# erwincoumans/tiny-differentiable-simulator

Measured on AMD Instinct MI355X. Metric: env-steps/sec, higher is better.
Workload: dtype f64

## Files before the change

tiny-differentiable-simulator_amd/csrc/tds_oct.hip:

```cpp
#include <hip/hip_runtime.h>
#include <stdlib.h>

#include "tds_device_model.h"
#include "tds_kernels.h"
#include "tds_lanes.h"
#include "tds_oct_windows.h"
#include "tds_step_shared.h"

#ifdef TDS_OCT_PROF
#ifndef TDS_OCT_PROF_WG
#define TDS_OCT_PROF_WG 3
#endif
__device__ unsigned long long tds_oct_prof_buf[64];
__device__ unsigned long long tds_oct_prof_clk[64];
__device__ unsigned long long tds_oct_prof_wg[3 * 2048];
__device__ int tds_oct_prof_iter = 500;
#define OCT_STAMP(k, pin)                                                                       \
  do {                                                                                          \
    unsigned long long t_;                                                                      \
    auto p_ = (pin);        \
    asm volatile("s_memtime %0\n\ts_waitcnt lgkmcnt(0)" : "=s"(t_), "+v"(p_)::"memory");        \
    if (prof_on) prof_t[k] = t_;                                                                \
  } while (0)
#define OCT_BAR_T(k)       \
  do {                     \
    OCT_STAMP(k, tid);     \
    OCT_BAR();             \
    OCT_STAMP((k) + 1, tid); \
  } while (0)
#define OCT_BAR_W(k, first)                                                                     \
  do {                                                                                          \
    unsigned long long a_, b_;                                                                  \
    asm volatile("s_memtime %0\n\ts_waitcnt lgkmcnt(0)" : "=s"(a_), "+v"(tid)::"memory");       \
    OCT_BAR();                                                                                  \
    asm volatile("s_memtime %0\n\ts_waitcnt lgkmcnt(0)" : "=s"(b_), "+v"(tid)::"memory");       \
    if (prof_on && (first)) {                                                                   \
      prof_t[k] = a_;                                                                           \
      prof_t[(k) + 1] = b_;                                                                     \
    } else if (prof_on) {                                                                       \
      prof_t[(k) + 2] += b_ - a_;                                                               \
    }                                                                                           \
  } while (0)
#else
#define OCT_STAMP(k, pin) do { } while (0)
#define OCT_BAR_T(k) OCT_BAR()
#define OCT_BAR_W(k, first) OCT_BAR()
#endif

#ifdef TDS_OCT_MARKS
#define OCT_MARK(name) asm volatile("; OCTMARK " name ::: "memory")
#else
#define OCT_MARK(name) do { } while (0)
#endif

#ifndef TDS_OCT_SD_LATE
#define TDS_OCT_SD_LATE 1
#endif
#ifndef TDS_OCT_CARRY
#define TDS_OCT_CARRY 1
#endif
#ifndef TDS_OCT_TOP_EARLY
#define TDS_OCT_TOP_EARLY 1
#endif
#ifndef TDS_OCT_SPLIT_LOOP
#define TDS_OCT_SPLIT_LOOP 0
#endif

namespace {

#define OCT_SYNC()                                             \
  do {                                                         \
    __builtin_amdgcn_fence(__ATOMIC_ACQ_REL, "wavefront");     \
    __builtin_amdgcn_wave_barrier();                           \
  } while (0)

template <int CTRL>
__device__ __forceinline__ double oct_dpp(double v) {
  const int l = __double2loint(v), h = __double2hiint(v);
  const int lo = __builtin_amdgcn_update_dpp(0, l, CTRL, 0xF, 0xF, true);
  const int hi = __builtin_amdgcn_update_dpp(0, h, CTRL, 0xF, 0xF, true);
  return __hiloint2double(hi, lo);
}
template <int CTRL>
__device__ __forceinline__ float oct_dpp(float v) {
  return __int_as_float(__builtin_amdgcn_update_dpp(0, __float_as_int(v), CTRL, 0xF, 0xF, true));
}
template <typename T>
__device__ __forceinline__ T pair_other(T v) { return oct_dpp<0xB1>(v); }
template <int K, typename T>
__device__ __forceinline__ T pair_bcast(T v) { return oct_dpp<(K == 0 ? 0xA0 : 0xF5)>(v); }
template <typename T>
__device__ __forceinline__ T oct_sum(T v) {
  asm volatile("" : "+v"(v));
  v += oct_dpp<0xB1>(v);
  v += oct_dpp<0x4E>(v);
  v += oct_dpp<0x141>(v);
  return v;
}
template <int K>
__device__ __forceinline__ double oct_bcast(double v) {
  const double t = __builtin_amdgcn_update_dpp(0.0, v, 0x150 + K, 0xF, 0x3, false);
  return __builtin_amdgcn_update_dpp(t, v, 0x150 + 8 + K, 0xF, 0xC, false);
}
template <int K>
__device__ __forceinline__ float oct_bcast(float v) {
  const int b = __float_as_int(v);
  const int t = __builtin_amdgcn_update_dpp(0, b, 0x150 + K, 0xF, 0x3, false);
  return __int_as_float(__builtin_amdgcn_update_dpp(t, b, 0x150 + 8 + K, 0xF, 0xC, false));
}

struct OctOff {
  int lcw, legf, swl, qdp, fac, win, xs, cp, stride;
};
struct OctLds {
  static constexpr int LCW = 6;
  static constexpr int ZW = 14;
  static constexpr int Z_B = 10, Z_A = 11, Z_G = 12, Z_HL = 13;
  static constexpr int NCP = 17;
};
__host__ __device__ inline OctOff oct_layout(int in_dim) {
  OctOff o;
  int at = in_dim + 4;
  at = (at + 1) & ~1;
  o.lcw = at;  at += 8 * OctLds::LCW;
  o.legf = at; at += 4 * 3;
  o.swl = at;  at += 8 * 6;
  o.qdp = at;  at += 8;
  o.fac = at;  at += 28;
  o.win = at;  at += 2 * 8 * OctLds::ZW;
  o.xs = at;   at += 3 * OctLds::NCP + 1;
  o.cp = at;   at += 5 * OctLds::NCP + 1;
  at = (at + 1) & ~1;
  while ((((at * 2) & 63) % 8) != 0 || ((at * 2) & 63) == 0 || ((at * 2) & 63) == 32) at += 2;
  o.stride = at;
  return o;
}

struct OctKernArgs {
  const void *mdl, *x_in;
  void *y_out;
  const void *actions;
  void *x_feedback, *obs_out;
  TdsStepCtl ctl;
  int n_envs;
  OctOff O;
};
using TB = TdsOctTab;
constexpr int TDS_OCT_PRIO = 1;

#define OCT_ST(v, p) (*(p) = (v))
#define OCT_BAR()                                                                        \
  do {                                                                                   \
    if constexpr (W2) asm volatile("s_waitcnt lgkmcnt(0)\n\ts_barrier" ::: "memory");    \
    else OCT_SYNC();                                                                     \
  } while (0)

template <typename T, typename TR, bool LOOP, int BUILD>
__device__ __forceinline__ void oct_body(const DevModel<T> *__restrict__ mdl_arg, const TR *x_in, TR *__restrict__ y_out,
                                         const TR *__restrict__ actions, TR *x_feedback ,
                                         TR *__restrict__ obs_out, const TdsStepCtl &ctl_arg, int n_envs, const OctOff &O) {
  extern __shared__ __align__(16) unsigned char tds_oct_smem[];
  T *const sm = reinterpret_cast<T *>(tds_oct_smem);
#ifdef TDS_OCT_PROF
  if (threadIdx.x == 0 && blockIdx.x < 2048) {
    unsigned long long c_;
    asm volatile("s_memrealtime %0\n\ts_waitcnt lgkmcnt(0)" : "=s"(c_)::"memory");
    tds_oct_prof_wg[3 * blockIdx.x] = c_;
  }
#endif
  constexpr bool W2 = BUILD >= 2;
  constexpr bool BATCH_SCHUR = LOOP && BUILD == 3;
  constexpr bool SD_LATE = LOOP && (BUILD == 2 || BUILD == 3) && TDS_OCT_SD_LATE != 0;
  constexpr bool CARRY = LOOP && BUILD == 3 && TDS_OCT_CARRY != 0;
  constexpr bool TOP_EARLY = LOOP && BUILD == 3 && TDS_OCT_TOP_EARLY != 0;
  constexpr bool SPLIT_LOOP = CARRY || TOP_EARLY || (LOOP && BUILD == 3 && TDS_OCT_SPLIT_LOOP != 0);
  constexpr int nq = 14, nd = 14, adim = 8, in_dim = nq + nd + adim + 3, w_obs = nq + nd + 2;
  constexpr int NT = W2 ? 128 : 64;
  T *const CT = sm + 8 * O.stride;
  {
    const int t = threadIdx.x;
    constexpr int TN = (TB::TOTAL + NT - 1) / NT, XN = (in_dim + 7) / 8;
    T tv[TN], xv[XN];
#pragma unroll
    for (int k = 0; k < TN; ++k) {
      const int i = t + k * NT;
      tv[k] = i < TB::TOTAL ? mdl_arg->oct_tab[i] : T(0);
    }
    const int lane0 = t & 7, grp0 = (t & 63) >> 3, env0 = blockIdx.x * 8 + grp0;
    const bool valid0 = env0 < n_envs && t < 64;
#pragma unroll
    for (int k = 0; k < XN; ++k) {
      const int i = lane0 + 8 * k;
      const bool act = actions != nullptr && i >= nq + nd && i < nq + nd + adim;
      xv[k] = (!valid0 || i >= in_dim) ? T(0) : act ? (T)actions[(size_t)env0 * adim + (i - nq - nd)] : (T)x_in[(size_t)env0 * in_dim + i];
    }
#pragma unroll
    for (int k = 0; k < TN; ++k) {
      const int i = t + k * NT;
      if (i < TB::TOTAL) CT[i] = tv[k];
    }
    if (t < 64) {
      T *const xr = sm + grp0 * O.stride;
#pragma unroll
      for (int k = 0; k < XN; ++k) {
        const int i = lane0 + 8 * k;
        if (i < in_dim) xr[i] = xv[k];
      }
      if (lane0 < 4) xr[in_dim + lane0] = T(0);
    }
    if constexpr (W2) __syncthreads();
    else OCT_SYNC();
  }
  const int nsteps = LOOP ? ctl_arg.nsub : 1;
  T next_act = T(0);
  int act_blk = 0, y_slot = 0, o_slot = 0;
  if constexpr (LOOP) {
    if (ctl_arg.act_pool != nullptr && ctl_arg.act_blocks > 0) act_blk = (ctl_arg.act_first + 1) % ctl_arg.act_blocks;
    if (ctl_arg.y_ring != nullptr && ctl_arg.y_slots > 0) y_slot = ctl_arg.y_first % ctl_arg.y_slots;
    if (ctl_arg.obs_ring != nullptr && ctl_arg.obs_slots > 0) o_slot = ctl_arg.obs_first % ctl_arg.obs_slots;
  }
  const int act_slot = (int)(CT + (threadIdx.x & 7) * TB::LSTR)[TB::ACT];
  struct Carried { T q, qd, rq[6], rqd[6]; };
  struct TopConsts { T S[6], rotf, nax[3], nn[6], xt[3], ipose, stiff, damp, act_lim, xt_ident, base_t[3], grav[3], kp, kd, max_force; };
  auto carry_load = [&](const T *xr_, int lane_, Carried &c) {
    c.q = xr_[6 + lane_];
    c.qd = xr_[nq + 6 + lane_];
#pragma unroll
    for (int r = 0; r < 6; ++r) {
      c.rq[r] = xr_[r];
      c.rqd[r] = xr_[nq + r];
    }
  };
  auto top_request = [&](const T *xr_, const T *CL_, TopConsts &t) {
#pragma unroll
    for (int k = 0; k < 6; ++k) t.S[k] = CL_[TB::S + k];
    t.rotf = CL_[TB::ROTF];
#pragma unroll
    for (int k = 0; k < 3; ++k) t.nax[k] = CL_[TB::NAX + k];
#pragma unroll
    for (int k = 0; k < 6; ++k) t.nn[k] = CL_[TB::NN + k];
#pragma unroll
    for (int k = 0; k < 3; ++k) t.xt[k] = CL_[TB::XT + 9 + k];
    t.ipose = CL_[TB::IPOSE];
    t.stiff = CL_[TB::STIFF];
    t.damp = CL_[TB::DAMP];
    t.act_lim = CT[TB::SC + TB::ACTION_LIMIT];
    t.xt_ident = CT[TB::SC + TB::XT_IDENT];
#pragma unroll
    for (int k = 0; k < 3; ++k) {
      t.base_t[k] = CT[TB::SC + TB::BASE_T + k];
      t.grav[k] = CT[TB::SC + TB::GRAV + k];
    }
    t.kp = xr_[nq + nd + adim];
    t.kd = xr_[nq + nd + adim + 1];
    t.max_force = xr_[nq + nd + adim + 2];
  };
  Carried car = {};
  TopConsts tc = {};
  if constexpr (CARRY || TOP_EARLY) {
    const int lane_ = threadIdx.x & 7;
    const T *const xr_ = sm + ((threadIdx.x & 63) >> 3) * O.stride;
    if constexpr (CARRY) carry_load(xr_, lane_, car);
    if constexpr (TOP_EARLY) top_request(xr_, CT + lane_ * TB::LSTR, tc);
  }
  auto step_body = [&](auto rolec, const int it) {
  constexpr int ROLE = decltype(rolec)::value;
  const __attribute__((address_space(4))) char *ka_seg = (const __attribute__((address_space(4))) char *)__builtin_amdgcn_kernarg_segment_ptr();
  int tid = threadIdx.x;
  if constexpr (LOOP) asm volatile("" : "+s"(ka_seg), "+v"(tid));
  const int wv = ROLE < 2 ? ROLE : (W2 ? __builtin_amdgcn_readfirstlane(tid >> 6) : 0);
  const bool is_main = !W2 || wv == 0, is_help = !W2 || wv == 1;
  if constexpr (W2 && TDS_OCT_PRIO != 0) {
    if (BUILD != 4 && wv == 0) __builtin_amdgcn_s_setprio(3);
    else __builtin_amdgcn_s_setprio(0);
  }
  (void)is_main;
  (void)is_help;
#ifdef TDS_OCT_PROF
  unsigned long long prof_t[56] = {};
  const bool prof_on = blockIdx.x == TDS_OCT_PROF_WG && it == tds_oct_prof_iter;
  if (it == 0 && tid == 0 && blockIdx.x < 2048) {
    unsigned long long c_;
    asm volatile("s_memrealtime %0\n\ts_waitcnt lgkmcnt(0)" : "=s"(c_)::"memory");
    tds_oct_prof_wg[3 * blockIdx.x + 1] = c_;
  }
  if (blockIdx.x == TDS_OCT_PROF_WG && it < 32 && tid == 0) {
    unsigned long long c0_, c1_;
    asm volatile("s_memtime %0\n\ts_memrealtime %1\n\ts_waitcnt lgkmcnt(0)" : "=s"(c0_), "=s"(c1_)::"memory");
    tds_oct_prof_clk[2 * it] = c0_;
    tds_oct_prof_clk[2 * it + 1] = c1_;
  }
#endif
  const int lane = tid & 7;
  const int grp = (tid & 63) >> 3;
  const int env = blockIdx.x * 8 + grp;
  const bool valid = env < n_envs;
  T *const E = sm + grp * O.stride;
  T *const xr = E;
  const int leg = lane >> 1, pos = lane & 1;
  const int dq = 6 + lane;
  const T *const CL = CT + lane * TB::LSTR;
  typename TdsCtlRef<LOOP>::type ctl = TdsCtlRef<LOOP>::get(ctl_arg, ka_seg + __builtin_offsetof(OctKernArgs, ctl));
  const T dt = CT[TB::SC + TB::DT];
  const int pgs_iters = (int)CT[TB::SC + TB::PGS_ITERATIONS];
  const bool last = it == nsteps - 1;
  OCT_STAMP(0, tid);

  T q, qd, tau;
  T Sl[6], R[9], p[3], sw[6], v[6], a0[6];
  T R5[9], P[3], A4[3], A5[3], pA3[3], pA4[3], pA5[3], v5[6], a5[6];
  T Lc[6], l10, id0, id1, sq0, sq1, my_id, my_sq, Ls[15], ids[6], sq_ids[6], qd_new, qdr_new[6];
  T Cb, Cr[6], It[10];
  T u = T(0), urm = T(0);
  T u_init = T(0), urm_init = T(0);
  T sw_mu = T(0), sw_rest = T(0), sw_cap = T(0), sw_hip = T(0);
  int na = 0, NA = 0;

  auto root_frame = [&](const T *rq, const T *bt, T sx, T cx, T sy, T cy, T sz, T cz) {
    R5[0] = cy * cz;                 R5[1] = -cy * sz;                R5[2] = sy;
    R5[3] = sx * sy * cz + cx * sz;  R5[4] = cx * cz - sx * sy * sz;  R5[5] = -sx * cy;
    R5[6] = sx * sz - cx * sy * cz;  R5[7] = cx * sy * sz + sx * cz;  R5[8] = cx * cy;
    P[0] = rq[0] + bt[0];
    P[1] = rq[1] + bt[1];
    P[2] = rq[2] + bt[2];
    A4[0] = T(0); A4[1] = cx; A4[2] = sx;
    A5[0] = sy; A5[1] = -sx * cy; A5[2] = cx * cy;
    pA3[0] = T(0); pA3[1] = P[2]; pA3[2] = -P[1];
    cross3(P, A4, pA4);
// ... 154 lines not shown
      }
      T Rl[9], pl[3], r[3];
      mat3_mul(Rq, Rp, Rl);
      mat3_mulv(Rq, tp, r);
#pragma unroll
      for (int k = 0; k < 3; ++k) pl[k] = pq[k] + r[k];
      mat3_mul(R5, Rl, R);
      mat3_mulv(R5, pl, r);
      p[0] = P[0] + r[0];
      p[1] = P[1] + r[1];
      p[2] = P[2] + r[2];
      mat3_mulv(R, Sl, sw);
      mat3_mulv(R, Sl + 3, sw + 3);
      T c[3];
      cross3(p, sw, c);
      sw[3] += c[0];
      sw[4] += c[1];
      sw[5] += c[2];
      T vJ[6];
#pragma unroll
      for (int k = 0; k < 6; ++k) vJ[k] = sw[k] * qd;
#pragma unroll
      for (int k = 0; k < 6; ++k) {
        const T sh = pair_bcast<0>(vJ[k]);
        v[k] = v5[k] + (vJ[k] + (take ? sh : T(0)));
      }
      T cb[6];
      cross3(v, vJ, cb);
      T c1[3], c2[3];
      cross3(v, vJ + 3, c1);
      cross3(v + 3, vJ, c2);
      cb[3] = c1[0] + c2[0];
      cb[4] = c1[1] + c2[1];
      cb[5] = c1[2] + c2[2];
#pragma unroll
      for (int k = 0; k < 6; ++k) {
        const T sh = pair_bcast<0>(cb[k]);
        a0[k] = a5[k] + (cb[k] + (take ? sh : T(0)));
      }
    }
    OCT_MARK("main_publish_kin");
    {
      T *const swl = E + O.swl + lane * 6;
#pragma unroll
      for (int k = 0; k < 6; ++k) swl[k] = sw[k];
      if constexpr (W2) {
        T *const kin = E + O.win + 8 * OctLds::ZW + lane * 12;
#pragma unroll
        for (int k = 0; k < 9; ++k) kin[k] = R[k];
#pragma unroll
        for (int k = 0; k < 3; ++k) kin[9 + k] = p[k];
      }
    }
    OCT_MARK("main_kin_end");
    OCT_STAMP(1, sw[5]);
  };

  const int ystr = ctl.y_stride;
  const int out_dim = (int)CT[TB::SC + TB::OUTPUT_DIM];
  const int nv = (int)CT[TB::SC + TB::NUM_VISUALS];
  auto y_where = [&](TR *&yo, TR *&yo2, int &yend, int &yend2) {
    int ys = y_slot;
    asm volatile("" : "+s"(ys));
    yo = nullptr;
    yo2 = nullptr;
    yend = ystr;
    yend2 = out_dim;
    if (LOOP && ctl.y_ring != nullptr) {
      yo = tds_global((TR *)ctl.y_ring) + ((size_t)ys * ctl.ring_envs + env) * ystr;
      if (last && y_out != nullptr) yo2 = y_out + (size_t)env * out_dim;
    } else if (last && y_out != nullptr) {
      yo = y_out + (size_t)env * (LOOP ? out_dim : ystr);
      yend = LOOP ? out_dim : ystr;
    }
  };
  unsigned sig_tok = 0u;

  auto help_np = [&]() {
    OCT_MARK("help_np");
    if constexpr (LOOP) {
      if (it > 0 && ctl.obs_ring != nullptr && ctl.peer_arrive != nullptr)
        sig_tok = tds_peer_count_in(ctl, (o_slot == 0 ? ctl.obs_slots : o_slot) - 1);
      if (ctl.act_pool != nullptr && it + 1 < nsteps && valid)
        next_act = (T)tds_global((const TR *)ctl.act_pool)[((size_t)act_blk * ctl.act_envs + env) * adim + lane];
    }
    if constexpr (W2) {
      const T *const kin = E + O.win + 8 * OctLds::ZW + lane * 12;
#pragma unroll
      for (int k = 0; k < 9; ++k) R[k] = kin[k];
#pragma unroll
      for (int k = 0; k < 3; ++k) p[k] = kin[9 + k];
      const T *const sc = E + O.win + 8 * OctLds::ZW + 96;
      root_frame(xr, CT + TB::SC + TB::BASE_T, sc[0], sc[1], sc[2], sc[3], sc[4], sc[5]);
    }
    {
      T *const cpx = E + O.cp;
      const T n[3] = {CT[TB::SC + TB::PLANE_N], CT[TB::SC + TB::PLANE_N + 1], CT[TB::SC + TB::PLANE_N + 2]};
      const T pc = CT[TB::SC + TB::PLANE_C];
      auto sphere = [&](const T *Rl, const T *pl, const T *loc, T rad, T *pt, T &dist) {
        T ctr[3];
        mat3_mulv(Rl, loc, ctr);
        ctr[0] += pl[0];
        ctr[1] += pl[1];
        ctr[2] += pl[2];
        const T t = -((-dot3(ctr, n)) + pc);
        dist = t - rad;
        pt[0] = ctr[0] - rad * n[0];
        pt[1] = ctr[1] - rad * n[1];
        pt[2] = ctr[2] - rad * n[2];
      };
      T pt0[3], pt1[3], ptt[3], d0, d1, dtt;
      sphere(R, p, CL + TB::CPL0, CL[TB::CPR0], pt0, d0);
      sphere(R, p, CL + TB::CPL1, CL[TB::CPR1], pt1, d1);
      sphere(R5, P, CT + TB::ROOT + TB::R_CPL, CT[TB::ROOT + TB::R_CPR], ptt, dtt);
      const bool act0 = valid && d0 < T(0), act1 = valid && d1 < T(0), actt = valid && dtt < T(0) && CT[TB::ROOT + TB::R_CPR] >= T(0);
      const unsigned long long b0 = __ballot(act0), b1 = __ballot(act1), bt = __ballot(actt);
      const unsigned m0 = (unsigned)((b0 >> (grp * 8)) & 0xFFull), m1 = (unsigned)((b1 >> (grp * 8)) & 0xFFull);
      const unsigned below = (1u << lane) - 1u;
      const int r0 = (actt ? 1 : 0) + __popc(m0 & below) + __popc(m1 & below);
      const int r1 = r0 + (act0 ? 1 : 0);
      if (act0) {
        cpx[0 * OctLds::NCP + r0] = pt0[0];
        cpx[1 * OctLds::NCP + r0] = pt0[1];
        cpx[2 * OctLds::NCP + r0] = pt0[2];
        cpx[3 * OctLds::NCP + r0] = d0;
        cpx[4 * OctLds::NCP + r0] = (T)lane;
      }
      if (act1) {
        cpx[0 * OctLds::NCP + r1] = pt1[0];
        cpx[1 * OctLds::NCP + r1] = pt1[1];
        cpx[2 * OctLds::NCP + r1] = pt1[2];
        cpx[3 * OctLds::NCP + r1] = d1;
        cpx[4 * OctLds::NCP + r1] = (T)lane;
      }
      if (actt && lane == 0) {
        cpx[0 * OctLds::NCP] = ptt[0];
        cpx[1 * OctLds::NCP] = ptt[1];
        cpx[2 * OctLds::NCP] = ptt[2];
        cpx[3 * OctLds::NCP] = dtt;
        cpx[4 * OctLds::NCP] = T(8);
      }
      na = (actt ? 1 : 0) + __popc(m0) + __popc(m1);
#pragma unroll
      for (int g = 0; g < 8; ++g) {
        const int c = __popc((unsigned)((b0 >> (g * 8)) & 0xFFull)) + __popc((unsigned)((b1 >> (g * 8)) & 0xFFull)) + (int)((bt >> (g * 8)) & 1ull);
        NA = c > NA ? c : NA;
      }
      if constexpr (W2) {
        if ((tid & 63) == 0) sm[in_dim + 3] = (T)NA;
      }
    }
    OCT_STAMP(8, na);
  };
  auto help_poses = [&]() {
    OCT_MARK("help_signal_poses");
    if constexpr (LOOP) {
      if (ctl.act_pool != nullptr && !last) xr[nq + nd + lane] = next_act;
      if (it > 0 && ctl.obs_ring != nullptr) {
        if (ctl.peer_arrive != nullptr) tds_peer_finish(ctl, (o_slot == 0 ? ctl.obs_slots : o_slot) - 1, sig_tok);
        else tds_signal_slot(ctl, (o_slot == 0 ? ctl.obs_slots : o_slot) - 1);
      }
    }
    TR *yo, *yo2;
    int yend, yend2;
    y_where(yo, yo2, yend, yend2);
    (void)yend;
    (void)yend2;
    if (valid && yo != nullptr && nv > 0) {
      auto pose_out = [&](const T *Rl, const T *pl, const T *vx, int k) {
        T Ro[9], po[3], qo[4];
        mat3_mul(Rl, vx, Ro);
        mat3_mulv(Rl, vx + 9, po);
        matrix_to_quat(Ro, qo);
        TR *o = yo + (nq + nd) + 7 * k;
        OCT_ST((TR)(pl[0] + po[0]), &o[0]);
        OCT_ST((TR)(pl[1] + po[1]), &o[1]);
        OCT_ST((TR)(pl[2] + po[2]), &o[2]);
        OCT_ST((TR)qo[0], &o[3]);
        OCT_ST((TR)qo[1], &o[4]);
        OCT_ST((TR)qo[2], &o[5]);
        OCT_ST((TR)qo[3], &o[6]);
        if (yo2 != nullptr) {
          TR *o2 = yo2 + (nq + nd) + 7 * k;
          OCT_ST((TR)(pl[0] + po[0]), &o2[0]);
          OCT_ST((TR)(pl[1] + po[1]), &o2[1]);
          OCT_ST((TR)(pl[2] + po[2]), &o2[2]);
          OCT_ST((TR)qo[0], &o2[3]);
          OCT_ST((TR)qo[1], &o2[4]);
          OCT_ST((TR)qo[2], &o2[5]);
          OCT_ST((TR)qo[3], &o2[6]);
        }
      };
      pose_out(R, p, CL + TB::VIS, 1 + lane);
      if (lane == 7) pose_out(R5, P, CT + TB::ROOT + TB::R_VIS, 0);
    }
    OCT_MARK("help_np_end");
    OCT_STAMP(9, na);
  };

  auto main_dyn = [&]() {
    auto rigid = [&](const T *Rl, const T *pl, T m, const T *com, const T *Ib, const T *vl, const T *al, T *Ic, T *fc) {
      T cw[3];
      mat3_mulv(Rl, com, cw);
      cw[0] += pl[0];
      cw[1] += pl[1];
      cw[2] += pl[2];
      T RI[9], Iw[9];
      mat3_mul(Rl, Ib, RI);
#pragma unroll
      for (int r = 0; r < 3; ++r)
#pragma unroll
        for (int c = 0; c < 3; ++c) Iw[3 * r + c] = RI[3 * r] * Rl[3 * c] + RI[3 * r + 1] * Rl[3 * c + 1] + RI[3 * r + 2] * Rl[3 * c + 2];
      const T c2 = dot3(cw, cw);
      Ic[0] = Iw[0] + m * (c2 - cw[0] * cw[0]);
      Ic[1] = T(0.5) * (Iw[1] + Iw[3]) - m * cw[0] * cw[1];
      Ic[2] = T(0.5) * (Iw[2] + Iw[6]) - m * cw[0] * cw[2];
      Ic[3] = Iw[4] + m * (c2 - cw[1] * cw[1]);
      Ic[4] = T(0.5) * (Iw[5] + Iw[7]) - m * cw[1] * cw[2];
      Ic[5] = Iw[8] + m * (c2 - cw[2] * cw[2]);
      Ic[6] = m * cw[0];
      Ic[7] = m * cw[1];
      Ic[8] = m * cw[2];
      Ic[9] = m;
      const T *const h = Ic + 6;
      T Iv[6], Ia[6], t3[3];
      sym3_mulv(Ic, vl, Iv);
      cross3(h, vl + 3, t3);
      Iv[0] += t3[0];
      Iv[1] += t3[1];
      Iv[2] += t3[2];
      cross3(h, vl, t3);
      Iv[3] = m * vl[3] - t3[0];
      Iv[4] = m * vl[4] - t3[1];
      Iv[5] = m * vl[5] - t3[2];
      sym3_mulv(Ic, al, Ia);
      cross3(h, al + 3, t3);
      Ia[0] += t3[0];
      Ia[1] += t3[1];
      Ia[2] += t3[2];
      cross3(h, al, t3);
      Ia[3] = m * al[3] - t3[0];
      Ia[4] = m * al[4] - t3[1];
      Ia[5] = m * al[5] - t3[2];
      T u3[3];
      cross3(vl, Iv, fc);
      cross3(vl + 3, Iv + 3, u3);
      fc[0] += u3[0];
      fc[1] += u3[1];
      fc[2] += u3[2];
      cross3(vl, Iv + 3, fc + 3);
#pragma unroll
      for (int k = 0; k < 6; ++k) fc[k] += Ia[k];
    };
    OCT_MARK("main_rigid");
    T Ic[10], fc[6];
    rigid(R, p, CL[TB::MASS], CL + TB::COM, CL + TB::INER, v, a0, Ic, fc);
    T ft[6];
    rigid(R5, P, CT[TB::ROOT + TB::R_MASS], CT + TB::ROOT + TB::R_COM, CT + TB::ROOT + TB::R_INER, v5, a5, It, ft);
    OCT_STAMP(2, ft[5]);
    OCT_MARK("main_totals");
#pragma unroll
    for (int k = 0; k < 10; ++k) It[k] += oct_sum(Ic[k]);
#pragma unroll
    for (int k = 0; k < 6; ++k) ft[k] += oct_sum(fc[k]);
    {
      const T recv = pos == 0 ? T(1) : T(0);
#pragma unroll
      for (int k = 0; k < 6; ++k) fc[k] += recv * pair_bcast<1>(fc[k]);
#pragma unroll
      for (int k = 0; k < 10; ++k) Ic[k] += recv * pair_bcast<1>(Ic[k]);
    }
    OCT_MARK("main_FC");
    T Fc[6];
    times_inertia(Ic, sw, Fc);
    Cb = dot6(sw, fc);
    const T ax3[6] = {T(1), T(0), T(0), pA3[0], pA3[1], pA3[2]}, ax4[6] = {A4[0], A4[1], A4[2], pA4[0], pA4[1], pA4[2]},
            ax5[6] = {A5[0], A5[1], A5[2], pA5[0], pA5[1], pA5[2]};
    Cr[0] = ft[3];
    Cr[1] = ft[4];
    Cr[2] = ft[5];
    Cr[3] = dot6(ax3, ft);
    Cr[4] = dot6(ax4, ft);
    Cr[5] = dot6(ax5, ft);
    T Bm0, Bm1, Cc[6];
    {
      T s0[6];
#pragma unroll
      for (int k = 0; k < 6; ++k) s0[k] = pair_bcast<0>(sw[k]);
      Bm0 = dot6(Fc, s0);
      Bm1 = dot6(Fc, sw);
      Cc[0] = Fc[3];
      Cc[1] = Fc[4];
      Cc[2] = Fc[5];
      Cc[3] = dot6(Fc, ax3);
      Cc[4] = dot6(Fc, ax4);
      Cc[5] = dot6(Fc, ax5);
    }
    OCT_MARK("main_legldl");
    {
      const T b00 = pair_bcast<0>(Bm0);
      const T b10 = pair_bcast<1>(Bm0), b11 = pair_bcast<1>(Bm1);
      sq0 = rsqrt_full<T>(b00);
      id0 = sq0 * sq0;
      l10 = b10 * id0;
      sq1 = rsqrt_full<T>(b11 - l10 * b10);
      id1 = sq1 * sq1;
    }
    my_id = pos == 0 ? id0 : id1;
    my_sq = pos == 0 ? sq0 : sq1;
    {
      T W[6];
      const T m1 = pos == 1 ? l10 : T(0);
#pragma unroll
      for (int r = 0; r < 6; ++r) {
        W[r] = Cc[r] - m1 * pair_bcast<0>(Cc[r]);
        Lc[r] = W[r] * my_id;
      }
      T *const lcw = E + O.lcw + lane * OctLds::LCW;
      T *const wl = E + O.xs + lane * 6;
#pragma unroll
      for (int r = 0; r < 6; ++r) {
        lcw[r] = Lc[r];
        wl[r] = W[r];
      }
      if (pos == 0) {
        T *const lf = E + O.legf + leg * 3;
        lf[0] = l10;
        lf[1] = sq0;
        lf[2] = sq1;
      }
    }
    OCT_STAMP(3, Lc[5]);
  };
  auto main_dyn2 = [&]() {
    OCT_MARK("main_schur");
    const T ax3[6] = {T(1), T(0), T(0), pA3[0], pA3[1], pA3[2]}, ax4[6] = {A4[0], A4[1], A4[2], pA4[0], pA4[1], pA4[2]},
            ax5[6] = {A5[0], A5[1], A5[2], pA5[0], pA5[1], pA5[2]};
    T Sm[21];
    T F3[6], F4[6];
    auto root_block_a1 = [&]() {
      const T m = It[9];
      times_inertia(It, ax3, F3);
      Sm[0] = m;
      Sm[1] = T(0); Sm[2] = m;
      Sm[3] = T(0); Sm[4] = T(0); Sm[5] = m;
      Sm[6] = F3[3]; Sm[7] = F3[4]; Sm[8] = F3[5]; Sm[9] = dot6(ax3, F3);
    };
    auto root_block_a2 = [&]() {
      times_inertia(It, ax4, F4);
      Sm[10] = F4[3]; Sm[11] = F4[4]; Sm[12] = F4[5]; Sm[13] = dot6(ax4, F3); Sm[14] = dot6(ax4, F4);
    };
    auto root_block_b = [&]() {
      T F5[6];
      times_inertia(It, ax5, F5);
      Sm[15] = F5[3]; Sm[16] = F5[4]; Sm[17] = F5[5]; Sm[18] = dot6(ax5, F3); Sm[19] = dot6(ax5, F4); Sm[20] = dot6(ax5, F5);
    };
    {
      const T *const lcw = E + O.lcw;
      const T *const wl = E + O.xs;
      T *const Ssum = E + O.fac;
      const int code = (int)CL[TB::SCHUR];
      if constexpr (BATCH_SCHUR) {
        T la[3][8], wa[3][8];
        int ee[3];
        auto ask = [&](auto pc) {
          constexpr int pass = decltype(pc)::value;
          const int rc = (code >> (6 * pass)) & 63;
          const int r = rc >> 3, rp = rc & 7;
          ee[pass] = (r * (r + 1)) / 2 + rp;
#pragma unroll
          for (int l = 0; l < 8; ++l) {
            la[pass][l] = lcw[l * OctLds::LCW + r];
            wa[pass][l] = wl[l * 6 + rp];
          }
        };
        auto sum = [&](auto pc) {
          constexpr int pass = decltype(pc)::value;
          T acc = T(0);
#pragma unroll
          for (int l = 0; l < 8; ++l) acc += la[pass][l] * wa[pass][l];
          Ssum[ee[pass]] = acc;
        };
        ask(std::integral_constant<int, 0>{});
        __builtin_amdgcn_sched_barrier(0);
        root_block_a1();
        __builtin_amdgcn_sched_barrier(0);
        sum(std::integral_constant<int, 0>{});
        ask(std::integral_constant<int, 1>{});
        __builtin_amdgcn_sched_barrier(0);
        root_block_a2();
        __builtin_amdgcn_sched_barrier(0);
        sum(std::integral_constant<int, 1>{});
        ask(std::integral_constant<int, 2>{});
        __builtin_amdgcn_sched_barrier(0);
        root_block_b();
        __builtin_amdgcn_sched_barrier(0);
        sum(std::integral_constant<int, 2>{});
      } else {
#pragma unroll
        for (int pass = 0; pass < 3; ++pass) {
          const int rc = (code >> (6 * pass)) & 63;
          const int r = rc >> 3, rp = rc & 7;
          const int e = (r * (r + 1)) / 2 + rp;
          T acc = T(0);
#pragma unroll
          for (int l = 0; l < 8; ++l) acc += lcw[l * OctLds::LCW + r] * wl[l * 6 + rp];
          Ssum[e] = acc;
        }
      }
    }
    OCT_MARK("main_Rblock");
    if constexpr (!BATCH_SCHUR) {
      root_block_a1();
      root_block_a2();
      root_block_b();
    }
    OCT_SYNC();
    OCT_MARK("main_ldl6");
    {
      const T *const Ssum = E + O.fac;
      if constexpr (BATCH_SCHUR) {
        T ss[21];
#pragma unroll
        for (int e = 0; e < 21; ++e) ss[e] = Ssum[e];
        __builtin_amdgcn_sched_barrier(0);
#pragma unroll
        for (int e = 0; e < 21; ++e) Sm[e] -= ss[e];
      } else {
#pragma unroll
        for (int e = 0; e < 21; ++e) Sm[e] -= Ssum[e];
      }
      static_for<0, 6>([&](auto kc) {
        constexpr int k = decltype(kc)::value;
        const T rs = rsqrt_full<T>(Sm[(k * (k + 1)) / 2 + k]);
        const T inv = rs * rs;
        sq_ids[k] = rs;
        ids[k] = inv;
        T col[6];
        static_for<k + 1, 6>([&](auto rc) {
          constexpr int r = decltype(rc)::value;
          col[r] = Sm[(r * (r + 1)) / 2 + k];
          Ls[(r * (r - 1)) / 2 + k] = col[r] * inv;
        });
        static_for<k + 1, 6>([&](auto rc) {
          constexpr int r = decltype(rc)::value;
          static_for<k + 1, r + 1>([&](auto cc) {
            constexpr int c = decltype(cc)::value;
            Sm[(r * (r + 1)) / 2 + c] -= Ls[(r * (r - 1)) / 2 + k] * col[c];
          });
        });
      });
    }
    OCT_STAMP(4, Ls[14]);
    OCT_MARK("main_fd");
    if constexpr (W2) {
      T *const fac = E + O.fac;
      OCT_SYNC();
      if (lane == 0) {
#pragma unroll
        for (int k = 0; k < 15; ++k) fac[k] = Ls[k];
#pragma unroll
        for (int k = 0; k < 6; ++k) fac[15 + k] = sq_ids[k];
      }
    }
    OCT_MARK("main_dyn_end");
  };
  auto main_fd = [&]() {
    OCT_MARK("main_fd");
    T y = tau - Cb;
    y -= (pos == 1 ? l10 : T(0)) * pair_bcast<0>(y);
    T yr[6];
#pragma unroll
    for (int r = 0; r < 6; ++r) yr[r] = -Cr[r] - oct_sum(Lc[r] * y);
    static_for<1, 6>([&](auto rc) {
      constexpr int r = decltype(rc)::value;
      static_for<0, r>([&](auto cc) {
        constexpr int c = decltype(cc)::value;
        yr[r] -= Ls[(r * (r - 1)) / 2 + c] * yr[c];
      });
    });
    u = -dt * (y * my_sq);
    T sel = yr[0] * sq_ids[0];
#pragma unroll
    for (int r = 1; r < 6; ++r) sel = lane == r ? yr[r] * sq_ids[r] : sel;
    urm = lane < 6 ? -dt * sel : T(0);
    u_init = u;
    urm_init = urm;
    OCT_STAMP(5, u);
  };
  auto main_sweep_consts = [&]() {
    OCT_SYNC();
    sw_mu = CT[TB::SC + TB::FRICTION];
    sw_rest = CT[TB::SC + TB::RESTITUTION];
    sw_hip = (T)(lane & ~1);
    int cap = 100000;
    asm volatile("" : "+v"(cap));
    sw_cap = (T)cap;
  };
  auto main_get_count = [&]() { NA = __builtin_amdgcn_readfirstlane((int)sm[in_dim + 3]); };
  auto help_get_factors = [&]() {
    const T *const fac = E + O.fac;
#pragma unroll
    for (int k = 0; k < 15; ++k) Ls[k] = fac[k];
#pragma unroll
    for (int k = 0; k < 6; ++k) sq_ids[k] = fac[15 + k];
  };

  struct RowRegs {
    T z0, z1, zr[6];
    int hl;
// ... 352 lines not shown
    OCT_MARK("main_pool_end");
    OCT_STAMP(7, tid);
  };
  auto help_rec = [&]() {
    OCT_MARK("help_rec");
    TR *yo, *yo2;
    int yend, yend2;
    y_where(yo, yo2, yend, yend2);
    if (valid && yo != nullptr && xr[in_dim + 3] == T(0)) {
      y_state(yo, yend);
      if (yo2 != nullptr) y_state(yo2, yend2);
    }
    if constexpr (LOOP) {
      if (ctl.obs_ring != nullptr) {
        const int slot = o_slot;
        const int rf = ctl.ring_flags;
        const bool f32w = (rf & TDS_RING_OBS_F32) != 0 || sizeof(TR) == 4;
        const int np = ctl.peer_arrive != nullptr ? ctl.n_peers : 0;
        const bool rd_only = (rf & TDS_RING_PEER_REWARD_DONE) != 0;
        if (ctl.peer_arrive != nullptr && (rf & TDS_RING_WIDE) != 0 && __all(valid)) {
          const int wl = tid & 63;
          const size_t row0 = ((size_t)slot * ctl.obs_envs + (size_t)blockIdx.x * 8) * (size_t)w_obs;
          const int per_unit = f32w ? 2 : 1;
          const int n_units = (8 * w_obs) / per_unit;
          const unsigned long long *const __attribute__((address_space(4))) *tab =
              (const unsigned long long *const __attribute__((address_space(4))) *)(const __attribute__((address_space(4))) void *)ctl.peer_ring;
          for (int u0 = 0; u0 < n_units; u0 += 64) {
            const int uu = u0 + wl;
            const bool on = uu < n_units;
            unsigned lo = 0u, hi = 0u;
            bool tail = false;
#pragma unroll
            for (int c = 0; c < 2; ++c) {
              if (c < per_unit) {
                const int f = on ? uu * per_unit + c : 0;
                const int e = f / w_obs;
                const int i = f - e * w_obs;
                const int src = i < nq + nd ? i : (i == nq + nd ? in_dim + 2 : in_dim + 1);
                const T vv = i < 2 ? T(0) : sm[e * O.stride + src];
                tail = tail || i >= nq + nd;
                if (f32w) {
                  const unsigned b = (unsigned)__float_as_int((float)vv);
                  if (c == 0) lo = b; else hi = b;
                } else {
                  const double dv = (double)vv;
                  lo = (unsigned)__double2loint(dv);
                  hi = (unsigned)__double2hiint(dv);
                }
              }
            }
            const unsigned long long bits = ((unsigned long long)hi << 32) | (unsigned long long)lo;
            const size_t unit_at = row0 / per_unit + (size_t)uu;
            if (on) __hip_atomic_store(tds_global((unsigned long long *)ctl.obs_ring) + unit_at, bits, __ATOMIC_RELAXED, __HIP_MEMORY_SCOPE_AGENT);
            const bool to_peers = on && (!rd_only || tail);
            for (int p0 = 0; p0 < np; p0 += 4) {
              const unsigned long long *const b0 = tds_global(tab[p0]), *const b1 = tds_global(tab[p0 + 1]), *const b2 = tds_global(tab[p0 + 2]),
                                       *const b3 = tds_global(tab[p0 + 3]);
              const size_t po = (size_t)ctl.peer_off / 8 + unit_at;
              if (to_peers) {
                using G64 = __attribute__((address_space(1))) unsigned long long;
                __hip_atomic_store((G64 *)((unsigned long long *)b0 + po), bits, __ATOMIC_RELAXED, __HIP_MEMORY_SCOPE_SYSTEM);
                if (p0 + 1 < np) __hip_atomic_store((G64 *)((unsigned long long *)b1 + po), bits, __ATOMIC_RELAXED, __HIP_MEMORY_SCOPE_SYSTEM);
                if (p0 + 2 < np) __hip_atomic_store((G64 *)((unsigned long long *)b2 + po), bits, __ATOMIC_RELAXED, __HIP_MEMORY_SCOPE_SYSTEM);
                if (p0 + 3 < np) __hip_atomic_store((G64 *)((unsigned long long *)b3 + po), bits, __ATOMIC_RELAXED, __HIP_MEMORY_SCOPE_SYSTEM);
              }
            }
          }
        } else if (valid) {
          const size_t at = ((size_t)slot * ctl.obs_envs + env) * w_obs;
          constexpr int NB = (w_obs + 7) / 8;
          T ov[NB];
#pragma unroll
          for (int k = 0; k < NB; ++k) {
            const int i = lane + 8 * k;
            const T rv = xr[i >= w_obs ? 0 : (i < nq + nd ? i : (i == nq + nd ? in_dim + 2 : in_dim + 1))];
            ov[k] = i < 2 ? T(0) : rv;
          }
#pragma unroll
          for (int k = 0; k < NB; ++k) {
            const int i = lane + 8 * k;
            if (i >= w_obs) continue;
            const T vv = ov[k];
            if (rf & TDS_RING_OBS_F32) {
              float *const pp = tds_global((float *)ctl.obs_ring) + at + i;
              if (rf & TDS_RING_NOFENCE) __hip_atomic_store(pp, (float)vv, __ATOMIC_RELAXED, __HIP_MEMORY_SCOPE_AGENT);
              else OCT_ST((float)vv, pp);
            } else {
              TR *const pp = tds_global((TR *)ctl.obs_ring) + at + i;
              if (rf & TDS_RING_NOFENCE) __hip_atomic_store(pp, (TR)vv, __ATOMIC_RELAXED, __HIP_MEMORY_SCOPE_AGENT);
              else OCT_ST((TR)vv, pp);
            }
            if (np > 0 && (i >= nq + nd || !rd_only)) {
              for (int pr = 0; pr < np; ++pr) {
                char *const pb = (char *)tds_global(((void *const __attribute__((address_space(4))) *)(const __attribute__((address_space(4))) void *)ctl.peer_ring)[pr]) + ctl.peer_off;
                if (rf & TDS_RING_OBS_F32) __hip_atomic_store((float *)pb + (at + i), (float)vv, __ATOMIC_RELAXED, __HIP_MEMORY_SCOPE_SYSTEM);
                else __hip_atomic_store((TR *)pb + (at + i), (TR)vv, __ATOMIC_RELAXED, __HIP_MEMORY_SCOPE_SYSTEM);
              }
            }
          }
        }
        if (last && ctl.peer_arrive != nullptr) tds_signal_slot(ctl, slot);
      }
    }
    if (valid && last) {
      for (int i = lane; i < nq + nd; i += 8) {
        const TR vv = (TR)xr[i];
        if (obs_out != nullptr) obs_out[(size_t)env * w_obs + i] = i < 2 ? TR(0) : vv;
        if (x_feedback != nullptr) x_feedback[(size_t)env * in_dim + i] = vv;
      }
      if (lane == 0 && obs_out != nullptr) {
        obs_out[(size_t)env * w_obs + nq + nd] = (TR)xr[in_dim + 2];
        obs_out[(size_t)env * w_obs + nq + nd + 1] = (TR)xr[in_dim + 1];
      }
    }
    OCT_MARK("help_rec_end");
    OCT_STAMP(11, tid);
  };

  if constexpr (W2) {
    if (wv == 0) {
      main_kin();
      OCT_BAR_T(24);
      main_dyn();
      OCT_BAR_T(26);
      main_dyn2();
      OCT_BAR_T(28);
      main_get_count();
      main_fd();
      main_sweep_consts();
      const int nr = 3 * NA;
      const bool lw = tds_oct_long_window(NA, 1, ctl.flags & TDS_CTL_OCT_LONG_WINDOW);
      int bo = 0;
      for (int pit = 0; pit < pgs_iters; ++pit) {
        for (int w0 = 0; w0 < nr;) {
          const int nw = tds_oct_main_windows(lw, pit, w0);
          OCT_BAR_W(30, (pit | w0) == 0);
          if ((pit | w0) == 0) OCT_STAMP(12, tid);
          if (pit == 0) main_sweep(std::true_type{}, w0, bo, nw == 2);
          else main_sweep(std::false_type{}, w0, bo, false);
          if ((pit | w0) == 0) OCT_STAMP(13, u);
          w0 += 8 * nw;
          if (nw == 1) bo = 8 * OctLds::ZW - bo;
        }
      }
      main_fin();
      main_pool();
      OCT_BAR_T(34);
    } else {
      OCT_BAR_T(40);
      help_np();
      RowRegs rw = {};
      if (NA > 0) rows_geom(0, 0, rw);
      OCT_BAR_T(42);
      if (NA > 0) {
        rows_leg(0, rw);
        rows_park(rw);
      }
      help_poses();
      if (NA > 0) rows_fetch(rw);
      OCT_BAR_T(44);
      if (tds_oct_help_has_windows(NA, pgs_iters)) {
        help_get_factors();
        rows_root(0, rw);
        OCT_BAR_W(46, true);
        const int nr = 3 * NA;
        int bo = 8 * OctLds::ZW;
        for (int pit = 0; pit < pgs_iters; ++pit) {
          for (int w0 = tds_oct_help_first_w0(pit); w0 < nr; w0 += 8) {
            rows_geom(w0, bo, rw);
            rows_leg(bo, rw);
            rows_root(bo, rw);
            OCT_BAR_W(46, false);
            bo = 8 * OctLds::ZW - bo;
          }
        }
      }
      OCT_BAR_T(50);
      help_rec();
    }
  } else {
    main_kin();
    OCT_SYNC();
    help_np();
    help_poses();
    main_dyn();
    OCT_SYNC();
    main_dyn2();
    main_fd();
    main_sweep_consts();
    const int nr = 3 * NA;
    int bo = 0;
    for (int pit = 0; pit < pgs_iters; ++pit) {
      for (int w0 = 0; w0 < nr; w0 += 8) {
        RowRegs rw;
        rows_geom(w0, bo, rw);
        rows_leg(bo, rw);
        rows_root(bo, rw);
        OCT_SYNC();
        if (pit == 0) main_sweep(std::true_type{}, w0, bo, false);
        else main_sweep(std::false_type{}, w0, bo, false);
        bo = 8 * OctLds::ZW - bo;
      }
    }
    main_fin();
    main_pool();
    OCT_SYNC();
    help_rec();
    if constexpr (LOOP) OCT_SYNC();
  }
#ifdef TDS_OCT_PROF
  if (prof_on && (tid & 63) == 0) {
#pragma unroll
    for (int k = 16; k < 24; ++k)
      if (is_main) tds_oct_prof_buf[k] = prof_t[k];
#pragma unroll
    for (int k = 0; k < 14; ++k)
      if (((k < 8 || k >= 12) && is_main) || (k >= 8 && k < 12 && is_help)) tds_oct_prof_buf[k] = prof_t[k];
    if (is_help) tds_oct_prof_buf[15] = (unsigned long long)NA;
#pragma unroll
    for (int k = 24; k < 36; ++k)
      if (is_main) tds_oct_prof_buf[k] = prof_t[k];
#pragma unroll
    for (int k = 40; k < 52; ++k)
      if (is_help) tds_oct_prof_buf[k] = prof_t[k];
  }
#endif
  if constexpr (LOOP) {
    act_blk = act_blk + 1 >= ctl_arg.act_blocks ? 0 : act_blk + 1;
    y_slot = y_slot + 1 >= ctl_arg.y_slots ? 0 : y_slot + 1;
    o_slot = o_slot + 1 >= ctl_arg.obs_slots ? 0 : o_slot + 1;
  }
  };
  if constexpr (SPLIT_LOOP) {
    if (__builtin_amdgcn_readfirstlane((int)threadIdx.x >> 6) == 0) {
      for (int it = 0; it < nsteps; ++it) step_body(std::integral_constant<int, 0>{}, it);
    } else {
      for (int it = 0; it < nsteps; ++it) step_body(std::integral_constant<int, 1>{}, it);
    }
  } else {
    for (int it = 0; it < nsteps; ++it) step_body(std::integral_constant<int, 2>{}, it);
  }
#ifdef TDS_OCT_PROF
  if (threadIdx.x == 0 && blockIdx.x < 2048) {
    unsigned long long c_;
    asm volatile("s_waitcnt vmcnt(0)\n\ts_memrealtime %0\n\ts_waitcnt lgkmcnt(0)" : "=s"(c_)::"memory");
    tds_oct_prof_wg[3 * blockIdx.x + 2] = c_;
  }
#endif
}

template <typename T, typename TR, bool LOOP, int BUILD>
__global__ __launch_bounds__(BUILD >= 2 ? 128 : 64) __attribute__((amdgpu_waves_per_eu(BUILD == 2 ? 2 : 1, BUILD == 2 ? 2 : 1)))
void tds_oct_kernel(const DevModel<T> *__restrict__ mdl_arg, const TR *x_in, TR *__restrict__ y_out,
                    const TR *__restrict__ actions, TR *x_feedback, TR *__restrict__ obs_out, TdsStepCtl ctl_arg, int n_envs,
                    OctOff O) {
  oct_body<T, TR, LOOP, BUILD>(mdl_arg, x_in, y_out, actions, x_feedback, obs_out, ctl_arg, n_envs, O);
}
template <typename T, typename TR, bool LOOP>
__global__ __launch_bounds__(128) __attribute__((amdgpu_waves_per_eu(2, 2), amdgpu_num_vgpr(120)))
void tds_oct_kernel_beside(const DevModel<T> *__restrict__ mdl_arg, const TR *x_in, TR *__restrict__ y_out,
                           const TR *__restrict__ actions, TR *x_feedback, TR *__restrict__ obs_out, TdsStepCtl ctl_arg,
                           int n_envs, OctOff O) {
  oct_body<T, TR, LOOP, 4>(mdl_arg, x_in, y_out, actions, x_feedback, obs_out, ctl_arg, n_envs, O);
}

}

#ifdef TDS_OCT_PROF
extern "C" int tds_oct_prof_workgroups(unsigned long long *out, int n_wg) {
  return hipMemcpyFromSymbol(out, HIP_SYMBOL(tds_oct_prof_wg), (size_t)3 * n_wg * sizeof(unsigned long long)) == hipSuccess ? 0 : -1;
}
extern "C" int tds_oct_prof_clocks(unsigned long long *out64) {
  return hipMemcpyFromSymbol(out64, HIP_SYMBOL(tds_oct_prof_clk), 64 * sizeof(unsigned long long)) == hipSuccess ? 0 : -1;
}
extern "C" int tds_oct_prof_read(unsigned long long *out64, int iter) {
  if (out64 && hipMemcpyFromSymbol(out64, HIP_SYMBOL(tds_oct_prof_buf), 64 * sizeof(unsigned long long)) != hipSuccess) return -1;
  if (iter >= 0 && hipMemcpyToSymbol(HIP_SYMBOL(tds_oct_prof_iter), &iter, sizeof(int)) != hipSuccess) return -1;
  return 0;
}
#endif

int tds_oct_lds_bytes(int input_dim) { return oct_layout(input_dim).stride * (int)sizeof(double); }
int tds_oct_workgroup_bytes(int input_dim) {
  return (oct_layout(input_dim).stride * 8 + TdsOctTab::TOTAL) * (int)sizeof(double);
}

template <typename T, typename TR>
int tds_launch_oct(const DevModel<T> *d_model, const DevModel<T> &h_model, const TR *x_in, TR *y_out, const TR *actions,
                   TR *x_feedback, TR *obs_out, int n_envs, hipStream_t stream, const TdsStepCtl &ctl, int build) {
  const OctOff O = oct_layout(h_model.input_dim);
  const int blocks = (n_envs + 7) / 8;
  const size_t shmem = ((size_t)O.stride * 8 + TdsOctTab::TOTAL) * sizeof(T);
  const bool one_step = ctl.nsub == 1 && ctl.obs_ring == nullptr && ctl.y_ring == nullptr;
#define OCT_LAUNCH(LOOP_, B_)                                                                                                 \
  hipLaunchKernelGGL((tds_oct_kernel<T, TR, LOOP_, B_>), dim3(blocks), dim3(B_ >= 2 ? 128 : 64), shmem, stream, d_model, x_in, \
                     y_out, actions, x_feedback, obs_out, ctl, n_envs, O)
  if (build == 4) {
    if (one_step)
      hipLaunchKernelGGL((tds_oct_kernel_beside<T, TR, false>), dim3(blocks), dim3(128), shmem, stream, d_model, x_in, y_out, actions,
                         x_feedback, obs_out, ctl, n_envs, O);
    else
      hipLaunchKernelGGL((tds_oct_kernel_beside<T, TR, true>), dim3(blocks), dim3(128), shmem, stream, d_model, x_in, y_out, actions,
                         x_feedback, obs_out, ctl, n_envs, O);
  } else if (one_step) {
    if (build == 3) OCT_LAUNCH(false, 3);
    else if (build == 2) OCT_LAUNCH(false, 2);
    else OCT_LAUNCH(false, 1);
  } else {
    if (build == 3) OCT_LAUNCH(true, 3);
    else if (build == 2) OCT_LAUNCH(true, 2);
    else OCT_LAUNCH(true, 1);
  }
#undef OCT_LAUNCH
  return (int)hipGetLastError();
}
template int tds_launch_oct<double, double>(const DevModel<double> *, const DevModel<double> &, const double *, double *,
                                            const double *, double *, double *, int, hipStream_t, const TdsStepCtl &, int);
template int tds_launch_oct<double, float>(const DevModel<double> *, const DevModel<double> &, const float *, float *,
                                           const float *, float *, float *, int, hipStream_t, const TdsStepCtl &, int);
```

Measured before the change: 657.9 million.

## Offload Schur accumulation to helper wave and defer pose output

The Schur-complement reduction over leg contributions moves from the main wave to the helper wave, with a new barrier pair so the main wave runs its root-block computations while the helper does the dot products. Pose output writes in the helper are split, so the signalling head runs early and the global pose stores are deferred until after the PGS window loop, and the rows_park/rows_fetch staging is dropped. The aim is better balance of critical-path work between the two wavefronts. The cost is an extra barrier and a different register and LDS timing profile for the helper.

```diff
diff --git a/tiny-differentiable-simulator_amd/csrc/tds_oct.hip b/tiny-differentiable-simulator_amd/csrc/tds_oct.hip
--- a/tiny-differentiable-simulator_amd/csrc/tds_oct.hip
+++ b/tiny-differentiable-simulator_amd/csrc/tds_oct.hip
@@ -65,6 +65,12 @@
 #ifndef TDS_OCT_SPLIT_LOOP
 #define TDS_OCT_SPLIT_LOOP 0
 #endif
+#ifndef TDS_OCT_POSES_LATE
+#define TDS_OCT_POSES_LATE 1
+#endif
+#ifndef TDS_OCT_HELP_SCHUR
+#define TDS_OCT_HELP_SCHUR 1
+#endif
 
 namespace {
 
@@ -174,6 +180,8 @@
   constexpr bool CARRY = LOOP && BUILD == 3 && TDS_OCT_CARRY != 0;
   constexpr bool TOP_EARLY = LOOP && BUILD == 3 && TDS_OCT_TOP_EARLY != 0;
   constexpr bool SPLIT_LOOP = CARRY || TOP_EARLY || (LOOP && BUILD == 3 && TDS_OCT_SPLIT_LOOP != 0);
+  constexpr bool POSES_LATE = LOOP && BUILD == 3 && TDS_OCT_POSES_LATE != 0;
+  constexpr bool HELP_SCHUR = LOOP && BUILD == 3 && TDS_OCT_HELP_SCHUR != 0;
   constexpr int nq = 14, nd = 14, adim = 8, in_dim = nq + nd + adim + 3, w_obs = nq + nd + 2;
   constexpr int NT = W2 ? 128 : 64;
   T *const CT = sm + 8 * O.stride;
@@ -634,7 +642,7 @@
     }
     OCT_STAMP(8, na);
   };
-  auto help_poses = [&]() {
+  auto help_poses_head = [&]() {
     OCT_MARK("help_signal_poses");
     if constexpr (LOOP) {
       if (ctl.act_pool != nullptr && !last) xr[nq + nd + lane] = next_act;
@@ -643,6 +651,9 @@
         else tds_signal_slot(ctl, (o_slot == 0 ? ctl.obs_slots : o_slot) - 1);
       }
     }
+  };
+  auto help_poses_tail = [&]() {
+    if constexpr (POSES_LATE) OCT_MARK("help_poses_late");
     TR *yo, *yo2;
     int yend, yend2;
     y_where(yo, yo2, yend, yend2);
@@ -678,6 +689,10 @@
     }
     OCT_MARK("help_np_end");
     OCT_STAMP(9, na);
+  };
+  auto help_poses = [&]() {
+    help_poses_head();
+    help_poses_tail();
   };
 
   auto main_dyn = [&]() {
@@ -814,6 +829,36 @@
     }
     OCT_STAMP(3, Lc[5]);
   };
+  auto help_schur = [&]() {
+    OCT_MARK("help_schur");
+    const T *const lcw = E + O.lcw;
+    const T *const wl = E + O.xs;
+    T *const Ssum = E + O.fac;
+    const int code = (int)CL[TB::SCHUR];
+    T la[3][8], wa[3][8];
+    int ee[3];
+#pragma unroll
+    for (int pass = 0; pass < 3; ++pass) {
+      const int rc = (code >> (6 * pass)) & 63;
+      const int r = rc >> 3, rp = rc & 7;
+      ee[pass] = (r * (r + 1)) / 2 + rp;
+#pragma unroll
+      for (int l = 0; l < 8; ++l) {
+        la[pass][l] = lcw[l * OctLds::LCW + r];
+        wa[pass][l] = wl[l * 6 + rp];
+      }
+    }
+    __builtin_amdgcn_sched_barrier(0);
+#pragma unroll
+    for (int pass = 0; pass < 3; ++pass) {
+      T acc = T(0);
+#pragma unroll
+      for (int l = 0; l < 8; ++l) acc += la[pass][l] * wa[pass][l];
+      Ssum[ee[pass]] = acc;
+    }
+    OCT_MARK("help_schur_end");
+    OCT_STAMP(14, na);
+  };
   auto main_dyn2 = [&]() {
     OCT_MARK("main_schur");
     const T ax3[6] = {T(1), T(0), T(0), pA3[0], pA3[1], pA3[2]}, ax4[6] = {A4[0], A4[1], A4[2], pA4[0], pA4[1], pA4[2]},
@@ -837,7 +882,15 @@
       times_inertia(It, ax5, F5);
       Sm[15] = F5[3]; Sm[16] = F5[4]; Sm[17] = F5[5]; Sm[18] = dot6(ax5, F3); Sm[19] = dot6(ax5, F4); Sm[20] = dot6(ax5, F5);
     };
-    {
+    if constexpr (HELP_SCHUR) {
+      __builtin_amdgcn_sched_barrier(0);
+      root_block_a1();
+      root_block_a2();
+      root_block_b();
+      __builtin_amdgcn_sched_barrier(0);
+      OCT_MARK("main_wait_schur");
+      OCT_BAR_T(36);
+    } else {
       const T *const lcw = E + O.lcw;
       const T *const wl = E + O.xs;
       T *const Ssum = E + O.fac;
@@ -1496,12 +1549,21 @@
       RowRegs rw = {};
       if (NA > 0) rows_geom(0, 0, rw);
       OCT_BAR_T(42);
-      if (NA > 0) {
-        rows_leg(0, rw);
-        rows_park(rw);
-      }
-      help_poses();
-      if (NA > 0) rows_fetch(rw);
+      if constexpr (HELP_SCHUR) {
+        help_schur();
+        OCT_BAR_T(52);
+      }
+      if constexpr (POSES_LATE) {
+        if (NA > 0) rows_leg(0, rw);
+        help_poses_head();
+      } else {
+        if (NA > 0) {
+          rows_leg(0, rw);
+          rows_park(rw);
+        }
+        help_poses();
+        if (NA > 0) rows_fetch(rw);
+      }
       OCT_BAR_T(44);
       if (tds_oct_help_has_windows(NA, pgs_iters)) {
         help_get_factors();
@@ -1519,6 +1581,7 @@
           }
         }
       }
+      if constexpr (POSES_LATE) help_poses_tail();
       OCT_BAR_T(50);
       help_rec();
     }
@@ -1561,11 +1624,12 @@
     for (int k = 0; k < 14; ++k)
       if (((k < 8 || k >= 12) && is_main) || (k >= 8 && k < 12 && is_help)) tds_oct_prof_buf[k] = prof_t[k];
     if (is_help) tds_oct_prof_buf[15] = (unsigned long long)NA;
-#pragma unroll
-    for (int k = 24; k < 36; ++k)
+    if (is_help) tds_oct_prof_buf[14] = prof_t[14];
+#pragma unroll
+    for (int k = 24; k < 38; ++k)
       if (is_main) tds_oct_prof_buf[k] = prof_t[k];
 #pragma unroll
-    for (int k = 40; k < 52; ++k)
+    for (int k = 40; k < 54; ++k)
       if (is_help) tds_oct_prof_buf[k] = prof_t[k];
   }
 #endif
```

Result: faster. 677.3 million, median of 6 (+3.0%).
